# kjeffery/SimplePath

Hardware: AMD Instinct MI355X
Metric: Mrays/sec (+ Msamples/sec) at fixed spp; per-pixel L2 vs CPU ref (higher is better)
Workload: dtype f32; 1 GPU; bunny.sp 1920x1080 @ 256 spp, direct_lighting; width=1920, height=1080, spp=256, integrator=direct_lighting, bvh=sah, tiles=32400, pipeline=megakernel, parallelism=tiles1

## Files before the change

simplepath_amd/csrc/common/sp_libm.h:

```cpp
#pragma once
#include "sp_math.h"
#include "sp_glibc_data.h"

namespace spm {

SP_HD double dfma(double a, double b, double c) { return __builtin_fma(a, b, c); }
SP_HD double gd(const uint64_t* t, int i) { return u2d(t[i]); }

template <uint64_t B>
SP_HD double vk(double dep)
{
#if defined(__HIP_DEVICE_COMPILE__)
    uint32_t lo, hi;
    asm("v_mov_b32 %0, %1 ; %2" : "=v"(lo) : "i"((uint32_t)(B & 0xffffffffull)), "v"(dep));
    asm("v_mov_b32 %0, %1 ; %2" : "=v"(hi) : "i"((uint32_t)(B >> 32)), "v"(dep));
    return u2d(((uint64_t)hi << 32) | (uint64_t)lo);
#else
    (void)dep;
    return u2d(B);
#endif
}

#if defined(__HIP_DEVICE_COMPILE__)
static __shared__ uint64_t lds_exp2f_t[32];
static __shared__ uint64_t lds_logf_t[32];
static __shared__ uint64_t lds_powf_t[32];
__device__ __forceinline__ void libm_lds_init(int tid, int nthreads)
{
    for (int i = tid; i < 32; i += nthreads) {
        lds_exp2f_t[i] = glibc::EXP2F_T[i];
        lds_logf_t[i]  = glibc::LOGF_T[i];
        lds_powf_t[i]  = glibc::POWF_T[i];
    }
}
#define SPM_EXP2F_T lds_exp2f_t
#define SPM_LOGF_T lds_logf_t
#define SPM_POWF_T lds_powf_t
#else
SP_HD void libm_lds_init(int, int) {}
#define SPM_EXP2F_T glibc::EXP2F_T
#define SPM_LOGF_T glibc::LOGF_T
#define SPM_POWF_T glibc::POWF_T
#endif
SP_HD float gf(const uint32_t* t, int i) { return u2f(t[i]); }

SP_HD float x86_default_nan() { return u2f(0xffc00000u); }
SP_HD float x86_quiet(float x) { return u2f(f2u(x) | 0x00400000u); }
SP_HD bool  is_nan_bits(float x) { return (f2u(x) & 0x7fffffffu) > 0x7f800000u; }
SP_HD float x86_add(float a, float b)
{
    if (is_nan_bits(a)) return x86_quiet(a);
    if (is_nan_bits(b)) return x86_quiet(b);
    return a + b;
}

SP_HD float lm_expf(float x)
{
#if defined(SP_XP_FASTLIBM) && defined(__HIP_DEVICE_COMPILE__)
    return __expf(x);
#endif
    using namespace glibc;
    const uint32_t ix     = f2u(x);
    const uint32_t abstop = (ix >> 20) & 0x7ffu;
    const double   xd     = (double)x;
    if (abstop > 0x42au) {
        if (ix == 0xff800000u) return 0.0f;
        if (abstop > 0x7f7u) return x86_add(x, x);
        if (x > gf(EXPF_LIM, 0)) return __builtin_inff();
        if (gf(EXPF_LIM, 1) > x) return 0.0f;
        if (!(gf(EXPF_LIM, 2) <= x)) return u2f(0x00000001u);
    }
    const double invln2n = gd(EXPF_K, 1), shift = gd(EXPF_K, 0);
    double       kd      = dfma(invln2n, xd, shift);
    const uint64_t ki    = d2u(kd);
    kd -= shift;
    const double r = dfma(invln2n, xd, -kd);
    uint64_t     t = SPM_EXP2F_T[ki & 31u] + (ki << 47);
    const double s  = u2d(t);
    const double z  = dfma(r, gd(EXPF_K, 2), vk<EXPF_K[3]>(r));
    const double r2 = r * r;
    double       y  = dfma(r, gd(EXPF_K, 4), gd(ONE_D, 0));
    y               = dfma(z, r2, y);
    y               = y * s;
    return (float)y;
}

SP_HD float lm_logf(float x)
{
#if defined(SP_XP_FASTLIBM) && defined(__HIP_DEVICE_COMPILE__)
    return __logf(x);
#endif
    using namespace glibc;
    uint32_t ix = f2u(x);
    if (ix == 0x3f800000u) return 0.0f;
    if (ix - 0x00800000u > 0x7effffffu) {
        if (ix * 2u == 0u) return -__builtin_inff();
        if (ix == 0x7f800000u) return x;
        if (ix * 2u > 0xfeffffffu) return x86_quiet(x);
        if (ix & 0x80000000u) return x86_default_nan();
        ix = f2u(x * gf(TWO23_F, 0)) - (23u << 23);
    }
    const uint32_t tmp  = ix - 0x3f330000u;
    const uint32_t i    = (tmp >> 19) & 15u;
    const int32_t  k    = (int32_t)tmp >> 23;
    const uint32_t iz   = ix - (tmp & 0xff800000u);
    const double   invc = gd(SPM_LOGF_T, 2 * i), logc = gd(SPM_LOGF_T, 2 * i + 1);
    const double   z    = (double)u2f(iz);
    const double   r    = dfma(z, invc, gd(MINUS_ONE_D, 0));
    const double   y0   = dfma((double)k, gd(LOGF_K, 0), logc);
    const double   r2   = r * r;
    double         y    = dfma(r, gd(LOGF_K, 2), vk<LOGF_K[3]>(r));
    y                   = dfma(r2, gd(LOGF_K, 1), y);
    y                   = dfma(r2, y, r + y0);
    return (float)y;
}

SP_HD int powf_checkint(uint32_t iy)
{
    const int e = (int)((iy >> 23) & 0xffu);
    if (e < 0x7f) return 0;
    if (e > 0x7f + 23) return 2;
    if (iy & ((1u << (0x7f + 23 - e)) - 1u)) return 0;
    if (iy & (1u << (0x7f + 23 - e))) return 1;
    return 2;
}
SP_HD bool powf_zeroinfnan(uint32_t ix) { return 2u * ix - 1u >= 2u * 0x7f800000u - 1u; }
SP_HD bool issignalingf(uint32_t ix) { return ((ix & 0x7fffffffu) > 0x7f800000u) && !(ix & 0x00400000u); }

SP_HD float lm_powf(float x, float y)
{
#if defined(SP_XP_FASTLIBM) && defined(__HIP_DEVICE_COMPILE__)
    return __powf(x, y);
#endif
    using namespace glibc;
    uint32_t       sign_bias = 0;
    uint32_t       ix = f2u(x);
    const uint32_t iy = f2u(y);
    if (ix - 0x00800000u >= 0x7f000000u || powf_zeroinfnan(iy)) {
        if (powf_zeroinfnan(iy)) {
            if (2u * iy == 0u) return issignalingf(ix) ? x86_add(x, y) : 1.0f;
            if (ix == 0x3f800000u) return issignalingf(iy) ? x86_add(x, y) : 1.0f;
            if (2u * ix > 2u * 0x7f800000u || 2u * iy > 2u * 0x7f800000u) return x86_add(x, y);
            if (2u * ix == 2u * 0x3f800000u) return 1.0f;
            if ((2u * ix < 2u * 0x3f800000u) == !(iy & 0x80000000u)) return 0.0f;
            return y * y;
        }
        if (powf_zeroinfnan(ix)) {
            float x2 = x * x;
            if ((ix & 0x80000000u) && powf_checkint(iy) == 1) x2 = -x2;
            return (iy & 0x80000000u) ? 1.0f / x2 : x2;
        }
        if (ix & 0x80000000u) {
            const int yint = powf_checkint(iy);
            if (yint == 0) return x86_default_nan();
            if (yint == 1) sign_bias = 1u << 16;
            ix &= 0x7fffffffu;
        }
        if (ix < 0x00800000u) {
            ix = f2u(x * gf(TWO23_F, 0)) & 0x7fffffffu;
            ix -= 23u << 23;
        }
    }
    const uint32_t tmp  = ix - 0x3f330000u;
    const uint32_t i    = (tmp >> 19) & 15u;
    const uint32_t top  = tmp & 0xff800000u;
    const uint32_t iz   = ix - top;
    const int32_t  k    = (int32_t)top >> 23;
    const double   invc = gd(SPM_POWF_T, 2 * i), logc = gd(SPM_POWF_T, 2 * i + 1);
    const double   z    = (double)u2f(iz);
    const double   r    = dfma(z, invc, gd(MINUS_ONE_D, 0));
    const double   y0   = (double)k + logc;
    const double   r2   = r * r;
    double         yy   = dfma(r, gd(POWF_A, 0), vk<POWF_A[1]>(r));
    const double   p    = dfma(r, gd(POWF_A, 2), vk<POWF_A[3]>(r));
    const double   r4   = r2 * r2;
    double         q    = dfma(r, gd(POWF_A, 4), y0);
    q                   = dfma(r2, p, q);
    yy                  = dfma(yy, r4, q);
    const double ylogx  = (double)y * yy;
    if (((d2u(ylogx) >> 47) & 0xffffu) > 0x80beu) {
        if (ylogx > gd(POWF_LIM, 0)) return sign_bias ? -__builtin_inff() : __builtin_inff();
        if (ylogx > gd(POWF_LIM, 1)) {
            const float one = gf(POWF_FLIM, 1) < 0.0f ? 1.0f : 1.0f;
            (void)one;
        }
        if (!(gd(POWF_LIM, 2) < ylogx)) return sign_bias ? -0.0f : 0.0f;
        if (!(gd(POWF_LIM, 3) <= ylogx)) return u2f(sign_bias ? 0x80000001u : 0x00000001u);
    }
    const double   shift = gd(EXP2F_K, 0);
    double         kd    = ylogx + shift;
    const uint64_t ki    = d2u(kd);
    kd -= shift;
    const double   rr  = ylogx - kd;
    uint64_t       t   = SPM_EXP2F_T[ki & 31u];
    const uint64_t ski = ki + sign_bias;
    t += ski << 47;
    const double s   = u2d(t);
    const double zz  = dfma(rr, gd(EXP2F_K, 1), vk<EXP2F_K[2]>(rr));
    const double rr2 = rr * rr;
    double       res = dfma(rr, gd(EXP2F_K, 3), gd(ONE_D, 0));
    res              = dfma(zz, rr2, res);
    res              = res * s;
    return (float)res;
}

SP_HD double sc(int k) { return gd(glibc::SINCOSF_T, k); }
enum { SC_HPI_INV = 4, SC_HPI = 5, SC_C0 = 6, SC_C1 = 7, SC_S1 = 8, SC_C2 = 9, SC_S2 = 10, SC_C3 = 11, SC_S3 = 12, SC_C4 = 13 };
SP_HD double sincos_sign(int q) { return (q == 1 || q == 2) ? -1.0 : 1.0; }

SP_HD float sincosf_poly(double x, double x2, int tab, int n)
{
    if ((n & 1) == 0) {
        const double s1 = dfma(x2, sc(SC_S3), vk<glibc::SINCOSF_T[SC_S2]>(x2));
        const double x3 = x2 * x;
        const double x7 = x2 * x3;
        const double s  = dfma(x3, sc(SC_S1), x);
        return (float)dfma(s1, x7, s);
    }
    const double x4 = x2 * x2;
    const double c1 = dfma(x2, sc(SC_C1), vk<glibc::SINCOSF_T[SC_C0]>(x2));
    const double c2 = dfma(x2, sc(SC_C4), vk<glibc::SINCOSF_T[SC_C3]>(x2));
    const double x6 = x2 * x4;
    const double c  = dfma(x4, sc(SC_C2), c1);
    const float  r  = (float)dfma(c2, x6, c);
    return tab ? -r : r;
}

SP_HD double sincosf_reduce_large(uint32_t xi, int* np)
{
    const uint32_t* arr   = glibc::INV_PIO4 + ((xi >> 26) & 15u);
    const int       shift = (int)((xi >> 23) & 7u);
    xi                    = (xi & 0xffffffu) | 0x800000u;
    xi <<= shift;
    uint64_t res0 = (uint64_t)(uint32_t)(xi * arr[0]);
    uint64_t res1 = (uint64_t)xi * arr[4];
    uint64_t res2 = (uint64_t)xi * arr[8];
    res0          = (res2 >> 32) | (res0 << 32);
    res0 += res1;
    const uint64_t n = (res0 + (1ull << 61)) >> 62;
    res0 -= n << 62;
    const double x = (double)(int64_t)res0;
    *np            = (int)n;
    return x * u2d(glibc::PI63[0]);
}

template <bool BOUNDED = false>
SP_HD float lm_sinf(float y)
{
#if defined(SP_XP_FASTLIBM) && defined(__HIP_DEVICE_COMPILE__)
    return __sinf(y);
#endif
    const uint32_t iy     = f2u(y);
    const uint32_t abstop = (iy >> 20) & 0x7ffu;
    double         x      = (double)y;
    if (abstop <= 0x3f3u) {
        const double s = x * x;
        if (abstop <= 0x397u) return y;
        return sincosf_poly(x, s, 0, 0);
    }
    if (BOUNDED || abstop <= 0x42eu) {
        const double r  = x * sc(SC_HPI_INV);
        int          n  = (((int32_t)r) + 0x800000) >> 24;
        x               = dfma(-(double)n, sc(SC_HPI), x);
        const double sg = sincos_sign(n & 3);
        const int    tb = (n & 2) ? 1 : 0;
        return sincosf_poly(x * sg, x * x, tb, n);
    }
    if (abstop <= 0x7f7u) {
        const int sign = (int)(iy >> 31);
        int       n;
        x               = sincosf_reduce_large(iy, &n);
        const double sg = sincos_sign((n + sign) & 3);
        const int    tb = ((n + sign) & 2) ? 1 : 0;
        return sincosf_poly(x * sg, x * x, tb, n);
    }
    return ((iy & 0x7fffffffu) > 0x7f800000u) ? x86_quiet(y) : x86_default_nan();
}

template <bool BOUNDED = false>
SP_HD float lm_cosf(float y)
{
#if defined(SP_XP_FASTLIBM) && defined(__HIP_DEVICE_COMPILE__)
    return __cosf(y);
#endif
    const uint32_t iy     = f2u(y);
    const uint32_t abstop = (iy >> 20) & 0x7ffu;
// ... 356 lines not shown
```

simplepath_amd/csrc/common/sp_math.h:

```cpp
#pragma once

#include <stdint.h>
#include <math.h>

#if defined(__HIPCC__)
#include <hip/hip_runtime.h>
#define SP_HD __host__ __device__ __forceinline__
#define SP_DEV __device__ __forceinline__
#else
#define SP_HD static inline
#define SP_DEV static inline
#endif

#if !defined(__HIP_DEVICE_COMPILE__)
#include <immintrin.h>
#endif

namespace spm {

SP_HD uint32_t f2u(float f) { return __builtin_bit_cast(uint32_t, f); }
SP_HD float u2f(uint32_t u) { return __builtin_bit_cast(float, u); }
SP_HD uint64_t d2u(double d) { return __builtin_bit_cast(uint64_t, d); }
SP_HD double u2d(uint64_t u) { return __builtin_bit_cast(double, u); }

SP_HD float std_max(float a, float b) { return (a < b) ? b : a; }
SP_HD float std_min(float a, float b) { return (b < a) ? b : a; }
SP_HD float std_clamp(float v, float lo, float hi) { return (v < lo) ? lo : ((hi < v) ? hi : v); }
SP_HD float sse_min(float a, float b) { return (a < b) ? a : b; }
SP_HD float sse_max(float a, float b) { return (a > b) ? a : b; }
SP_HD float fma_f(float a, float b, float c) { return __builtin_fmaf(a, b, c); }
SP_HD float abs_f(float a) { return __builtin_fabsf(a); }
SP_HD float sqrt_f(float a) { return __builtin_sqrtf(a); }
SP_HD float copysign_f(float a, float b) { return __builtin_copysignf(a, b); }

constexpr float k_pi          = 3.14159265358979323846f;
constexpr float k_inv_pi      = 0.318309886183790671538f;
constexpr float k_ray_epsilon = 0.001f;
constexpr float k_infinite    = 3.40282346638528859812e+38f;

struct RsqrtTable {
    const uint32_t* entries;
    int32_t         bits;
    uint32_t        zero_result;
    uint32_t        denorm_result;
    int32_t  pack_shift = 0;
    uint32_t pack_hi    = 0;
};

SP_HD float rsqrtss_emulated(float x, const RsqrtTable& t)
{
    const uint32_t u = f2u(x);
    const uint32_t e = (u >> 23) & 0xffu;
    if ((u >> 31) != 0u) {
        if ((u & 0x7fffffffu) == 0u) return u2f(0xff800000u);
        if (e == 0xffu && (u & 0x7fffffu) != 0u) return u2f(u | 0x400000u);
        return u2f(0xffc00000u);
    }
    if (e == 0xffu) {
        if ((u & 0x7fffffu) != 0u) return u2f(u | 0x400000u);
        return 0.0f;
    }
    if (e == 0u) {
        if (u == 0u) return u2f(t.zero_result);
        return u2f(t.denorm_result);
    }
    const int32_t  ex   = (int32_t)e - 127;
    const int32_t  p    = ex & 1;
    const int32_t  q    = (ex - p) / 2;
    const uint32_t m    = (u & 0x7fffffu) >> (23 - t.bits);
    const uint32_t i    = ((uint32_t)p << t.bits) | m;
    const uint32_t r    = t.pack_shift ? (t.pack_hi | ((uint32_t)((const uint16_t*)t.entries)[i] << t.pack_shift)) : t.entries[i];
    const int32_t  re   = (int32_t)((r >> 23) & 0xffu) - q;
    return u2f((r & 0x807fffffu) | ((uint32_t)re << 23));
}

SP_HD float rsqrt_newton(float a, float r)
{
    const float t1 = 1.5f * r;
    const float t2 = a * -0.5f;
    const float t3 = t2 * r;
    const float t4 = r * r;
    const float t5 = t3 * t4;
    return t1 + t5;
}

#if !defined(__HIP_DEVICE_COMPILE__)
static inline float rsqrtss_host(float x) { return _mm_cvtss_f32(_mm_rsqrt_ss(_mm_set_ss(x))); }
#else
static inline float rsqrtss_host(float) { return 0.0f; }
#endif

struct f3 {
    float x, y, z;
};

SP_HD f3 mk(float x, float y, float z) { f3 r; r.x = x; r.y = y; r.z = z; return r; }
SP_HD f3 add(f3 a, f3 b) { return mk(a.x + b.x, a.y + b.y, a.z + b.z); }
SP_HD f3 sub(f3 a, f3 b) { return mk(a.x - b.x, a.y - b.y, a.z - b.z); }
SP_HD f3 mul(f3 a, f3 b) { return mk(a.x * b.x, a.y * b.y, a.z * b.z); }
SP_HD f3 scale(f3 a, float s) { return mk(a.x * s, a.y * s, a.z * s); }
SP_HD f3 scale(float s, f3 a) { return mk(s * a.x, s * a.y, s * a.z); }
SP_HD f3 divs(f3 a, float s) { return mk(a.x / s, a.y / s, a.z / s); }
SP_HD f3 neg(f3 a) { return mk(-a.x, -a.y, -a.z); }
SP_HD f3 madd(f3 a, f3 b, f3 c) { return mk(fma_f(a.x, b.x, c.x), fma_f(a.y, b.y, c.y), fma_f(a.z, b.z, c.z)); }
SP_HD f3 madd(float a, f3 b, f3 c) { return mk(fma_f(a, b.x, c.x), fma_f(a, b.y, c.y), fma_f(a, b.z, c.z)); }

SP_HD float dot(f3 a, f3 b)
{
    const float p0 = a.x * b.x;
    const float p1 = a.y * b.y;
    const float p2 = a.z * b.z;
    return (p0 + p1) + (p2 + 0.0f);
}

SP_HD float dop1(float a, float b, float c, float d)
{
    const float cd  = c * d;
    const float err = fma_f(-c, d, cd);
    const float dop = fma_f(a, b, -cd);
    return dop + err;
}

SP_HD f3 cross(f3 a, f3 b)
{
    return mk(dop1(a.y, b.z, a.z, b.y), dop1(a.z, b.x, a.x, b.z), dop1(a.x, b.y, a.y, b.x));
}

SP_HD float length(f3 a) { return sqrt_f(dot(a, a)); }

struct rgb {
    float r, g, b;
};
SP_HD rgb mkc(float r, float g, float b) { rgb c; c.r = r; c.g = g; c.b = b; return c; }
SP_HD rgb cadd(rgb a, rgb b) { return mkc(a.r + b.r, a.g + b.g, a.b + b.b); }
SP_HD rgb csub(rgb a, rgb b) { return mkc(a.r - b.r, a.g - b.g, a.b - b.b); }
SP_HD rgb cmul(rgb a, rgb b) { return mkc(a.r * b.r, a.g * b.g, a.b * b.b); }
SP_HD rgb cscale(rgb a, float s) { return mkc(a.r * s, a.g * s, a.b * s); }
SP_HD rgb cdivs(rgb a, float s) { return mkc(a.r / s, a.g / s, a.b / s); }
SP_HD bool cblack(rgb a) { return a.r == 0.0f && a.g == 0.0f && a.b == 0.0f; }
SP_HD float luminance(rgb c) { return 0.2126f * c.r + 0.7152f * c.g + 0.0722f * c.b; }

struct aff {
    f3 vx, vy, vz, p;
};
struct lin {
    f3 vx, vy, vz;
};

SP_HD f3 xfm_point(const aff& m, f3 p)
{
    return madd(mk(p.x, p.x, p.x), m.vx, madd(mk(p.y, p.y, p.y), m.vy, madd(mk(p.z, p.z, p.z), m.vz, m.p)));
}
SP_HD f3 xfm_vector(const f3& vx, const f3& vy, const f3& vz, f3 a)
{
    return madd(mk(a.x, a.x, a.x), vx, madd(mk(a.y, a.y, a.y), vy, mul(mk(a.z, a.z, a.z), vz)));
}
// ... 5 lines not shown
```

simplepath_amd/csrc/hip/sp_path.hpp:

```cpp
#pragma once
#include "sp_device.hpp"

namespace spd {
inline namespace SPD_LAYOUT_NS {

using namespace spm;

#ifdef SP_WAVE_PROF
static __shared__ unsigned long long wprof_lds[16 * 16];
__device__ __forceinline__ void wprof_end(int k, uint64_t t0)
{
    const uint64_t dt    = __builtin_amdgcn_s_memtime() - t0;
    const uint64_t m     = __ballot(1);
    const int      first = __ffsll((unsigned long long)m) - 1;
    if ((int)(threadIdx.x & 63) == first) {
        const int w = threadIdx.x >> 6;
        wprof_lds[w * 16 + 2 * k] += dt;
        wprof_lds[w * 16 + 2 * k + 1] += dt * (uint64_t)__popcll(m);
    }
}
#define SP_WPROF(k, stmt)                                                                                              \
    do {                                                                                                               \
        const uint64_t t_wp_ = __builtin_amdgcn_s_memtime();                                                           \
        stmt;                                                                                                          \
// ... 1529 lines not shown
    lm_sincosf_bounded(phi, &sp, &cp);
    return mk(r * cp, y, r * sp);
}
__device__ __forceinline__ P2 concentric_disk(P2 u)
{
    constexpr float pi_over_4 = k_pi / 4.0f;
    constexpr float pi_over_2 = k_pi / 2.0f;
    const float     ox = 2.0f * u.x - 1.0f;
    const float     oy = 2.0f * u.y - 1.0f;
    P2              r;
    if (ox == 0.0f && oy == 0.0f) { r.x = 0.0f; r.y = 0.0f; return r; }
    float theta, rad;
    if (abs_f(ox) > abs_f(oy)) { rad = ox; theta = pi_over_4 * (oy / ox); }
    else { rad = oy; theta = pi_over_2 - pi_over_4 * (ox / oy); }
    float st, ct;
    lm_sincosf_bounded(theta, &st, &ct);
    r.x = rad * ct;
    r.y = rad * st;
    return r;
}
__device__ __forceinline__ f3 sample_cosine_hemisphere(P2 u)
{
    const P2    d = concentric_disk(u);
    const float y = sqrt_unit(std_max(0.0f, 1.0f - d.x * d.x - d.y * d.y));
    return mk(d.x, y, d.y);
}
constexpr float k_uniform_sphere_pdf     = 1.0f / (4.0f * k_pi);
constexpr float k_uniform_hemisphere_pdf = 1.0f / (2.0f * k_pi);

struct Onb {
    f3 u, v, w;
};
__device__ __forceinline__ Onb onb_of_unit(f3 v)
{
    const float sign = copysign_f(1.0f, v.z);
    const float a    = -1.0f / (sign + v.z);
    const float b    = v.x * v.y * a;
    const f3    b1   = mk(1.0f + sign * v.x * v.x * a, sign * b, -sign * v.x);
    const f3    b2   = mk(b, sign + v.y * v.y * a, -v.y);
    Onb         o;
    o.u = b2;
    o.v = v;
    o.w = b1;
    return o;
}
__device__ __forceinline__ Onb onb_from_v(f3 n, const Rsq& q) { return onb_of_unit(normalize(n, q)); }
__device__ __forceinline__ f3 to_world(const Onb& o, f3 a) { return add(add(scale(a.x, o.u), scale(a.y, o.v)), scale(a.z, o.w)); }
__device__ __forceinline__ f3 to_onb(const Onb& o, f3 a) { return mk(dot(a, o.u), dot(a, o.v), dot(a, o.w)); }

struct MSample {
    rgb   color;
    f3    dir;
    float pdf;
    int   props;
};
constexpr int PROP_DIFFUSE = 1, PROP_GLOSSY = 2, PROP_SPECULAR = 4, PROP_REFLECTIVE = 8;

__device__ __forceinline__ float cos2_theta(f3 w) { return w.y * w.y; }
__device__ __forceinline__ float sin2_theta(f3 w) { return std_max(0.0f, 1.0f - cos2_theta(w)); }
__device__ __forceinline__ float sin_theta(f3 w) { return sqrt_unit(sin2_theta(w)); }
__device__ __forceinline__ float tan_theta(f3 w) { return sin_theta(w) / w.y; }
__device__ __forceinline__ float tan2_theta(f3 w) { return sin2_theta(w) / cos2_theta(w); }
__device__ __forceinline__ float cos_phi(f3 w)
{
    const float st = sin_theta(w);
    return (st == 0.0f) ? 1.0f : std_clamp(w.x / st, -1.0f, 1.0f);
}
__device__ __forceinline__ float sin_phi(f3 w)
{
    const float st = sin_theta(w);
    return (st == 0.0f) ? 1.0f : std_clamp(w.z / st, -1.0f, 1.0f);
}
__device__ __forceinline__ bool same_hemisphere(f3 a, f3 b) { return a.y * b.y > 0.0f; }

__device__ __forceinline__ float fresnel_dielectric(float cos_i, float eta_i, float eta_t)
{
    cos_i = std_clamp(cos_i, -1.0f, 1.0f);
    if (!(cos_i > 0.0f)) {
        const float s = eta_i; eta_i = eta_t; eta_t = s;
        cos_i = abs_f(cos_i);
    }
    const float sin_i = sqrt_unit(std_max(0.0f, 1.0f - cos_i * cos_i));
    const float sin_t = eta_i / eta_t * sin_i;
    if (sin_t >= 1) return 1.0f;
    const float cos_t = sqrt_unit(std_max(0.0f, 1.0f - sin_t * sin_t));
    const float parl  = ((eta_t * cos_i) - (eta_i * cos_t)) / ((eta_t * cos_i) + (eta_i * cos_t));
    const float perp  = ((eta_i * cos_i) - (eta_t * cos_t)) / ((eta_i * cos_i) + (eta_t * cos_t));
    return (parl * parl + perp * perp) / 2.0f;
}

__device__ __forceinline__ float erfinv(float a)
{
    float       p;
    const float t = lm_logf(fma_f(a, 0.0f - a, 1.0f));
    if (abs_f(t) > 6.125f) {
        p = 3.03697567e-10f;
        p = fma_f(p, t, 2.93243101e-8f);
        p = fma_f(p, t, 1.22150334e-6f);
        p = fma_f(p, t, 2.84108955e-5f);
        p = fma_f(p, t, 3.93552968e-4f);
        p = fma_f(p, t, 3.02698812e-3f);
        p = fma_f(p, t, 4.83185798e-3f);
        p = fma_f(p, t, -2.64646143e-1f);
        p = fma_f(p, t, 8.40016484e-1f);
    } else {
        p = 5.43877832e-9f;
        p = fma_f(p, t, 1.43285448e-7f);
        p = fma_f(p, t, 1.22774793e-6f);
        p = fma_f(p, t, 1.12963626e-7f);
        p = fma_f(p, t, -5.61530760e-5f);
        p = fma_f(p, t, -1.47697632e-4f);
        p = fma_f(p, t, 2.31468678e-3f);
        p = fma_f(p, t, 1.15392581e-2f);
        p = fma_f(p, t, -2.32015476e-1f);
        p = fma_f(p, t, 8.86226892e-1f);
    }
    return a * p;
}

__device__ __forceinline__ P2 beckmann_sample11(float cos_theta_i, float U1, float U2)
{
    P2 s;
    if (cos_theta_i > .9999f) {
        const float r  = sqrt_f(-lm_logf(1.0f - U1));
        float       sp, cp;
        lm_sincosf_bounded(2.0f * k_pi * U2, &sp, &cp);
        s.x = r * cp;
        s.y = r * sp;
        return s;
    }
    const float sin_theta_i = sqrt_unit(std_max(0.0f, 1.0f - cos_theta_i * cos_theta_i));
    const float tan_theta_i = sin_theta_i / cos_theta_i;
    const float cot_theta_i = 1.0f / tan_theta_i;
    float       a           = -1.0f;
    float       c           = lm_erff(cot_theta_i);
    const float sample_x    = std_max(U1, 1e-6f);
    const float theta_i     = lm_acosf(cos_theta_i);
    const float fit         = 1.0f + theta_i * (-0.876f + theta_i * (0.4265f - 0.0594f * theta_i));
    float       b           = c - (1.0f + c) * lm_powf(1.0f - sample_x, fit);
    const float sqrt_pi_inv = 1.0f / sqrt_f(k_pi);
    const float normalization =
        1.0f / (1.0f + c + sqrt_pi_inv * tan_theta_i * lm_expf(-cot_theta_i * cot_theta_i));
#pragma unroll 1
    for (int it = 0; it < 9; ++it) {
        if (!(b >= a && b <= c)) b = 0.5f * (a + c);
        const float inv_erf = erfinv(b);
        const float value =
            normalization * (1.0f + b + sqrt_pi_inv * tan_theta_i * lm_expf(-inv_erf * inv_erf)) - sample_x;
        const float derivative = normalization * (1.0f - inv_erf * tan_theta_i);
        if (abs_f(value) < 1e-5f) break;
        if (value > 0) c = b;
        else a = b;
        b -= value / derivative;
    }
    s.x = erfinv(b);
    s.y = erfinv(2.0f * std_max(U2, 1e-6f) - 1.0f);
    return s;
}

__device__ __forceinline__ f3 beckmann_sample(f3 wi, float ax, float ay, float U1, float U2, const Rsq& q)
{
    const f3 st = normalize(mk(ax * wi.x, wi.y, ay * wi.z), q);
    P2       sl = beckmann_sample11(st.y, U1, U2);
    const float tmp = cos_phi(st) * sl.x - sin_phi(st) * sl.y;
    sl.y            = sin_phi(st) * sl.x + cos_phi(st) * sl.y;
    sl.x            = tmp;
    sl.x            = ax * sl.x;
    sl.y            = ay * sl.y;
    return normalize(mk(-sl.x, 1.0f, -sl.y), q);
}

__device__ __forceinline__ float beck_D(const Material& m, f3 wh)
{
    const float t2 = tan2_theta(wh);
    if (__builtin_isinf(t2)) return 0.0f;
    const float c4 = cos2_theta(wh) * cos2_theta(wh);
    const float cp = cos_phi(wh), sp = sin_phi(wh);
    return lm_expf(-t2 * ((cp * cp) / (m.alpha_x * m.alpha_x) + (sp * sp) / (m.alpha_y * m.alpha_y))) /
           (k_pi * m.alpha_x * m.alpha_y * c4);
}
__device__ __forceinline__ float beck_lambda(const Material& m, f3 w)
{
    const float at = abs_f(tan_theta(w));
    if (__builtin_isinf(at)) return 0.0f;
    const float cp    = cos_phi(w), sp = sin_phi(w);
    const float alpha = sqrt_f((cp * cp) * (m.alpha_x * m.alpha_x) + (sp * sp) * (m.alpha_y * m.alpha_y));
    const float a     = 1.0f / (alpha * at);
    if (a >= 1.6f) return 0.0f;
    return (1.0f - 1.259f * a + 0.396f * (a * a)) / (3.535f * a + 2.181f * (a * a));
}
__device__ __forceinline__ float beck_G1(const Material& m, f3 w) { return 1.0f / (1.0f + beck_lambda(m, w)); }
__device__ __forceinline__ float beck_G(const Material& m, f3 wo, f3 wi) { return 1.0f / (1.0f + beck_lambda(m, wo) + beck_lambda(m, wi)); }
__device__ __forceinline__ float beck_pdf(const Material& m, f3 wo, f3 wh)
{
    if (m.sample_visible_area) return beck_D(m, wh) * beck_G1(m, wo) * abs_f(dot(wo, wh)) / abs_f(wo.y);
    return beck_D(m, wh) * abs_f(wh.y);
}
__device__ __forceinline__ f3 beck_sample_wh(const Material& m, f3 wo, Rng& rng, const Rsq& q)
{
    const bool flip = wo.y < 0.0f;
    const float U2 = next1D(rng);
    const float U1 = next1D(rng);
    f3 wh = beckmann_sample(flip ? neg(wo) : wo, m.alpha_x, m.alpha_y, U1, U2, q);
    if (flip) wh = neg(wh);
    return wh;
}

__device__ __forceinline__ rgb mf_eval(const Material& m, f3 wo, f3 wi, const Rsq& q)
{
    const float ao = abs_f(wo.y), ai = abs_f(wi.y);
    if (ai == 0.0f || ao == 0.0f) return mkc(0, 0, 0);
    f3 wh = add(wi, wo);
    if (wh.x == 0.0f && wh.y == 0.0f && wh.z == 0.0f) return mkc(0, 0, 0);
    wh            = normalize(wh, q);
    const float f = fresnel_dielectric(dot(wi, wh), 1.0f, m.microfacet_ior);
    return cdivs(cscale(cscale(cscale(m.microfacet_r, beck_D(m, wh)), beck_G(m, wo, wi)), f), 4.0f * ai * ao);
}
__device__ __forceinline__ float mf_pdf(const Material& m, f3 wo, f3 wi, const Rsq& q)
{
    if (!same_hemisphere(wo, wi)) return 0.0f;
    const f3 wh = normalize(add(wo, wi), q);
    return beck_pdf(m, wo, wh) / (4.0f * dot(wo, wh));
}
__device__ __forceinline__ MSample mf_sample(const Material& m, f3 wo, Rng& rng, const Rsq& q)
{
    MSample r;
    r.color = mkc(0, 0, 0);
    r.dir   = mk(0, 0, 0);
    r.pdf   = 0.0f;
    r.props = 0;
    if (wo.y == 0.0f) return r;
    const f3    wh = beck_sample_wh(m, wo, rng, q);
    const float dp = dot(wo, wh);
    if (dp < 0.0f) return r;
    const f3 wi = add(neg(wo), scale(2.0f * dot(wo, wh), wh));
    if (!same_hemisphere(wo, wi)) return r;
    r.pdf   = beck_pdf(m, wo, wh) / (4.0f * dp);
    r.color = mf_eval(m, wo, wi, q);
    r.dir   = wi;
    r.props = PROP_GLOSSY | PROP_REFLECTIVE;
    return r;
}
struct BeckPre {
    bool  flip, steep;
    f3    st;
    float cphi, sphi;
    float tan_theta_i, c0, fit, normalization, sqrt_pi_inv;
    float lam_wo;
};
__device__ __forceinline__ BeckPre beck_pre(const Material& m, f3 wo, const Rsq& q)
{
    BeckPre p;
    p.flip               = wo.y < 0.0f;
    const f3 wi          = p.flip ? neg(wo) : wo;
    p.st                 = normalize(mk(m.alpha_x * wi.x, wi.y, m.alpha_y * wi.z), q);
    p.cphi               = cos_phi(p.st);
    p.sphi               = sin_phi(p.st);
    const float cos_t    = p.st.y;
    p.steep              = cos_t > .9999f;
    p.tan_theta_i = p.c0 = p.fit = p.normalization = p.sqrt_pi_inv = 0.0f;
    if (!p.steep) {
        const float sin_theta_i = sqrt_unit(std_max(0.0f, 1.0f - cos_t * cos_t));
        p.tan_theta_i           = sin_theta_i / cos_t;
        const float cot_theta_i = 1.0f / p.tan_theta_i;
        p.c0                    = lm_erff(cot_theta_i);
        const float theta_i     = lm_acosf(cos_t);
        p.fit                   = 1.0f + theta_i * (-0.876f + theta_i * (0.4265f - 0.0594f * theta_i));
        p.sqrt_pi_inv           = 1.0f / sqrt_f(k_pi);
        p.normalization = 1.0f / (1.0f + p.c0 + p.sqrt_pi_inv * p.tan_theta_i * lm_expf(-cot_theta_i * cot_theta_i));
    }
    p.lam_wo = beck_lambda(m, wo);
    return p;
}
__device__ __forceinline__ P2 beckmann_sample11_pre(const BeckPre& p, float U1, float U2)
{
    P2 s;
    if (p.steep) {
        const float r  = sqrt_f(-lm_logf(1.0f - U1));
        float       sp, cp;
        lm_sincosf_bounded(2.0f * k_pi * U2, &sp, &cp);
        s.x = r * cp;
        s.y = r * sp;
        return s;
    }
    float       a        = -1.0f;
    float       c        = p.c0;
    const float sample_x = std_max(U1, 1e-6f);
    float       b        = c - (1.0f + c) * lm_powf(1.0f - sample_x, p.fit);
    float inv_erf   = 0.0f;
    bool  converged = false;
#if defined(SP_WAVE_PROF) && defined(SP_WPROF_NEWTON)
    const uint64_t t_nl = __builtin_amdgcn_s_memtime();
#endif
#pragma unroll 1
    for (int it = 0; it < 9; ++it) {
#if defined(SP_WAVE_PROF) && defined(SP_WPROF_NEWTON)
        const uint64_t t_it = __builtin_amdgcn_s_memtime();
#endif
        if (!(b >= a && b <= c)) b = 0.5f * (a + c);
        inv_erf = erfinv(b);
        const float value =
            p.normalization * (1.0f + b + p.sqrt_pi_inv * p.tan_theta_i * lm_expf(-inv_erf * inv_erf)) - sample_x;
        const float derivative = p.normalization * (1.0f - inv_erf * p.tan_theta_i);
#if defined(SP_WAVE_PROF) && defined(SP_WPROF_NEWTON)
        wprof_end(4, t_it);
#endif
        if (abs_f(value) < 1e-5f) {
            converged = true;
            break;
        }
        if (value > 0) c = b;
        else a = b;
        b -= value / derivative;
    }
#if defined(SP_WAVE_PROF) && defined(SP_WPROF_NEWTON)
    wprof_end(5, t_nl);
#endif
    s.x = converged ? inv_erf : erfinv(b);
    s.y = erfinv(2.0f * std_max(U2, 1e-6f) - 1.0f);
    return s;
}
__device__ __forceinline__ MSample mf_sample_pre_u(const Material& m, const BeckPre& p, f3 wo, uint64_t u2, uint64_t u1,
                                                   const Rsq& q);
template <bool NT = false, bool PAIR = (SP_RNG_PAIR != 0)>
__device__ __forceinline__ MSample mf_sample_pre(const Material& m, const BeckPre& p, f3 wo, Rng& rng, const Rsq& q)
{
    MSample r;
    r.color = mkc(0, 0, 0);
    r.dir   = mk(0, 0, 0);
    r.pdf   = 0.0f;
    r.props = 0;
    if (wo.y == 0.0f) return r;
    uint64_t u2, u1;
    rng_raw2<NT, PAIR>(rng, u2, u1);
    return mf_sample_pre_u(m, p, wo, u2, u1, q);
}
struct MGeom {
    f3    dir;
    float pdf;
    float D, G, F, den;
    bool  valid;
    bool  black;
};
__device__ __forceinline__ MGeom mf_sample_geom(const Material& m, const BeckPre& p, f3 wo, uint64_t u2, uint64_t u1,
                                                const Rsq& q)
{
    MGeom g;
    g.dir   = mk(0, 0, 0);
    g.pdf   = 0.0f;
    g.D = g.G = g.F = 0.0f;
    g.den   = 1.0f;
    g.valid = false;
    g.black = true;
    const float U2 = canonical_from_u64(u2);
    const float U1 = canonical_from_u64(u1);
    P2          sl = beckmann_sample11_pre(p, U1, U2);
    const float tmp = p.cphi * sl.x - p.sphi * sl.y;
    sl.y            = p.sphi * sl.x + p.cphi * sl.y;
    sl.x            = tmp;
    sl.x            = m.alpha_x * sl.x;
    sl.y            = m.alpha_y * sl.y;
    f3 wh = normalize(mk(-sl.x, 1.0f, -sl.y), q);
    if (p.flip) wh = neg(wh);
    const float dp = dot(wo, wh);
    if (dp < 0.0f) return g;
    const f3 wi = add(neg(wo), scale(2.0f * dot(wo, wh), wh));
    if (!same_hemisphere(wo, wi)) return g;
    const float bpdf = m.sample_visible_area ? beck_D(m, wh) * (1.0f / (1.0f + p.lam_wo)) * abs_f(dot(wo, wh)) / abs_f(wo.y)
                                             : beck_D(m, wh) * abs_f(wh.y);
    g.pdf   = bpdf / (4.0f * dp);
    g.dir   = wi;
    g.valid = true;
    const float ao = abs_f(wo.y), ai = abs_f(wi.y);
    if (ai == 0.0f || ao == 0.0f) return g;
    f3 h = add(wi, wo);
    if (h.x == 0.0f && h.y == 0.0f && h.z == 0.0f) return g;
    h       = normalize(h, q);
    g.F     = fresnel_dielectric(dot(wi, h), 1.0f, m.microfacet_ior);
    g.G     = 1.0f / (1.0f + p.lam_wo + beck_lambda(m, wi));
    g.D     = beck_D(m, h);
    g.den   = 4.0f * ai * ao;
    g.black = false;
    return g;
}
__device__ __forceinline__ float mf_geom_channel(const MGeom& g, float R) { return g.black ? 0.0f : (((R * g.D) * g.G) * g.F) / g.den; }
__device__ __forceinline__ MSample mf_sample_pre_u(const Material& m, const BeckPre& p, f3 wo, uint64_t u2, uint64_t u1,
                                                   const Rsq& q)
{
    const MGeom g = mf_sample_geom(m, p, wo, u2, u1, q);
    MSample     r;
    r.color = mkc(0, 0, 0);
    r.dir   = g.dir;
    r.pdf   = g.pdf;
    r.props = 0;
    if (!g.valid) return r;
    r.color = mkc(mf_geom_channel(g, m.microfacet_r.r), mf_geom_channel(g, m.microfacet_r.g), mf_geom_channel(g, m.microfacet_r.b));
    r.props = PROP_GLOSSY | PROP_REFLECTIVE;
    return r;
}
__device__ __forceinline__ void rho_accumulate(rgb& r, const MGeom& g, rgb R, bool grey)
{
    if (!(g.pdf > 0.0f)) return;
    const float ay = abs_f(g.dir.y);
    r.r = r.r + (mf_geom_channel(g, R.r) * ay) / g.pdf;
    if (!grey) {
        r.g = r.g + (mf_geom_channel(g, R.g) * ay) / g.pdf;
        r.b = r.b + (mf_geom_channel(g, R.b) * ay) / g.pdf;
    }
}
#ifndef SP_RHO_ALIGNED
#define SP_RHO_ALIGNED 0
#endif
#ifndef SP_RHO_GREY
#define SP_RHO_GREY 1
#endif
template <bool PAIR = (SP_RNG_PAIR != 0), bool ALIGN = (SP_RHO_ALIGNED != 0), bool TOUCH = (SP_RHO_TOUCH != 0)>
__device__ __forceinline__ rgb mf_rho16(const Material& m, f3 wo, Rng& rng, const Rsq& q)
{
    const BeckPre p = beck_pre(m, wo, q);
    rgb           r = mkc(0, 0, 0);
    const bool grey = SP_RHO_GREY && f2u(m.microfacet_r.r) == f2u(m.microfacet_r.g) && f2u(m.microfacet_r.r) == f2u(m.microfacet_r.b);
    rng_reserve(rng, 32);
#if SP_RHO_TOUCH
    if constexpr (TOUCH) rng_touch(rng, 32, (__attribute__((address_space(3))) void*)rho_rng_sink);
#endif
    if constexpr (ALIGN && MT_BLK % 2 == 0 && RNG_PF == 0 && !SP_XP_SERVED_FREE) {
        if (wo.y == 0.0f) return cdivs(r, (float)16u);
        const int       odd   = rng.idx & 1;
        const uint64_t* cur   = mt_buf(rng, rng.cur);
        const uint64_t* next  = mt_buf(rng, mt_next(rng));
        uint64_t        carry = odd ? cur[mt_off(rng.idx)] : 0ull;
        for (unsigned i = 0; i < 16u; ++i) {
            const int       t = rng.idx + odd + 2 * (int)i;
            const uint64_t* b = (t < MT_N) ? cur + mt_off(t) : next + mt_off(t - MT_N);
            SP_TD(td_lines(rng.td_cat, b, 16));
            const ulonglong2 w  = *reinterpret_cast<const ulonglong2*>(b);
            const uint64_t   w0 = odd ? carry : w.x, w1 = odd ? w.x : w.y;
            carry               = w.y;
            rho_accumulate(r, mf_sample_geom(m, p, wo, mt_temper(w0), mt_temper(w1), q), m.microfacet_r, grey);
        }
        rng_skip_reserved(rng, 32);
        if (grey) r.g = r.b = r.r;
        return cdivs(r, (float)16u);
    }
    for (unsigned i = 0; i < 16u; ++i) {
        if (wo.y == 0.0f) continue;
        uint64_t u2, u1;
        rng_raw2<true, PAIR>(rng, u2, u1);
        rho_accumulate(r, mf_sample_geom(m, p, wo, u2, u1, q), m.microfacet_r, grey);
    }
    if (grey) r.g = r.b = r.r;
    return cdivs(r, (float)16u);
}

#if SP_SERVE_RHO
#ifndef SP_MERGE_QUERIES
#define SP_MERGE_QUERIES 1
#endif
enum : int {
    MQ_O = 0,
    MQ_D3 = 192,
    MQ_T3 = 384,
    MQ_D1 = 448,
    MQ_T1 = 640,
    MQ_BEST = 704,
    MQ_ANY = 832,
    MQ_TB = 896,
    MQ_Q = 960,
    MQ_CNT = 992,
    MQ_WORDS = 996,
    SRV_W = 0, SRV_REQ = 512, SRV_WORDS = 576,
    SRV_WAVE_WORDS = (SP_MERGE_QUERIES && MQ_WORDS > SRV_WORDS) ? MQ_WORDS : SRV_WORDS
};
static_assert(SRV_WAVE_WORDS % 4 == 0 && MQ_BEST % 2 == 0, "u64 LDS atomics need 8-byte alignment");
struct MqLayout {
    enum : int { O = MQ_O, D3 = MQ_D3, T3 = MQ_T3, D1 = MQ_D1, T1 = MQ_T1, BEST = MQ_BEST, AMAX = MQ_BEST, ANY = MQ_ANY,
                 TB = MQ_TB, Q = MQ_Q, CNT = MQ_CNT };
};
#ifndef SP_MQ_SHADOW
#define SP_MQ_SHADOW 1
#endif
static __shared__ __attribute__((aligned(16))) uint32_t srv_lds[4][SRV_WAVE_WORDS];
__device__ __forceinline__ float*   srv_w_at(int wave, int k, int j) { return reinterpret_cast<float*>(&srv_lds[wave][SRV_W + (k * 2 + j) * 64]); }
__device__ __forceinline__ uint8_t* srv_req_of(int wave) { return reinterpret_cast<uint8_t*>(&srv_lds[wave][SRV_REQ]); }
#endif

template <bool PAIR = (SP_RNG_PAIR != 0), bool ALIGN = (SP_RHO_ALIGNED != 0), bool TOUCH = (SP_RHO_TOUCH != 0)>
__device__ __forceinline__ void glossy_weights(const Material& m, f3 wo, Rng& rng, const Rsq& q, float w[2])
{
#if SP_SERVE_RHO
// ... 1007 lines not shown
```

Before: 3737 Mrays/s.

## Make libm and microfacet BSDF paths branchless and add unit-range powf fast path

Rewrites expf, logf, powf and the sqrt table lookup so the main polynomial path always runs, with special-case fixups moved to a rarely taken, expect-annotated tail. It also turns early returns in the Beckmann/Fresnel/microfacet eval, pdf, sample and rho helpers into computed selects, to reduce wavefront divergence. A new lm_powf_unit skips all special-case handling for the Beckmann sampling call sites, where x lies in (0,1). The cost is that every lane now does the full arithmetic even on paths that used to exit early, and the unchecked powf is correct only when the inputs stay in that range.

```diff
diff --git a/simplepath_amd/csrc/common/sp_libm.h b/simplepath_amd/csrc/common/sp_libm.h
--- a/simplepath_amd/csrc/common/sp_libm.h
+++ b/simplepath_amd/csrc/common/sp_libm.h
@@ -63,13 +63,6 @@
     const uint32_t ix     = f2u(x);
     const uint32_t abstop = (ix >> 20) & 0x7ffu;
     const double   xd     = (double)x;
-    if (abstop > 0x42au) {
-        if (ix == 0xff800000u) return 0.0f;
-        if (abstop > 0x7f7u) return x86_add(x, x);
-        if (x > gf(EXPF_LIM, 0)) return __builtin_inff();
-        if (gf(EXPF_LIM, 1) > x) return 0.0f;
-        if (!(gf(EXPF_LIM, 2) <= x)) return u2f(0x00000001u);
-    }
     const double invln2n = gd(EXPF_K, 1), shift = gd(EXPF_K, 0);
     double       kd      = dfma(invln2n, xd, shift);
     const uint64_t ki    = d2u(kd);
@@ -82,24 +75,20 @@
     double       y  = dfma(r, gd(EXPF_K, 4), gd(ONE_D, 0));
     y               = dfma(z, r2, y);
     y               = y * s;
-    return (float)y;
-}
-
-SP_HD float lm_logf(float x)
-{
-#if defined(SP_XP_FASTLIBM) && defined(__HIP_DEVICE_COMPILE__)
-    return __logf(x);
-#endif
-    using namespace glibc;
-    uint32_t ix = f2u(x);
-    if (ix == 0x3f800000u) return 0.0f;
-    if (ix - 0x00800000u > 0x7effffffu) {
-        if (ix * 2u == 0u) return -__builtin_inff();
-        if (ix == 0x7f800000u) return x;
-        if (ix * 2u > 0xfeffffffu) return x86_quiet(x);
-        if (ix & 0x80000000u) return x86_default_nan();
-        ix = f2u(x * gf(TWO23_F, 0)) - (23u << 23);
-    }
+    float res       = (float)y;
+    if (__builtin_expect(abstop > 0x42au, 0)) {
+        if (!(gf(EXPF_LIM, 2) <= x)) res = u2f(0x00000001u);
+        if (gf(EXPF_LIM, 1) > x) res = 0.0f;
+        if (x > gf(EXPF_LIM, 0)) res = __builtin_inff();
+        if (abstop > 0x7f7u) res = is_nan_bits(x) ? x86_quiet(x) : x + x;
+        if (ix == 0xff800000u) res = 0.0f;
+    }
+    return res;
+}
+
+SP_HD float logf_core(uint32_t ix)
+{
+    using namespace glibc;
     const uint32_t tmp  = ix - 0x3f330000u;
     const uint32_t i    = (tmp >> 19) & 15u;
     const int32_t  k    = (int32_t)tmp >> 23;
@@ -114,6 +103,24 @@
     y                   = dfma(r2, y, r + y0);
     return (float)y;
 }
+SP_HD float lm_logf(float x)
+{
+#if defined(SP_XP_FASTLIBM) && defined(__HIP_DEVICE_COMPILE__)
+    return __logf(x);
+#endif
+    using namespace glibc;
+    const uint32_t ix = f2u(x);
+    float          res = logf_core(ix);
+    res                = (ix == 0x3f800000u) ? 0.0f : res;
+    if (__builtin_expect(ix - 0x00800000u > 0x7effffffu, 0)) {
+        res = logf_core(f2u(x * gf(TWO23_F, 0)) - (23u << 23));
+        if (ix & 0x80000000u) res = x86_default_nan();
+        if (ix * 2u > 0xfeffffffu) res = x86_quiet(x);
+        if (ix == 0x7f800000u) res = x;
+        if (ix * 2u == 0u) res = -__builtin_inff();
+    }
+    return res;
+}
 
 SP_HD int powf_checkint(uint32_t iy)
 {
@@ -127,40 +134,42 @@
 SP_HD bool powf_zeroinfnan(uint32_t ix) { return 2u * ix - 1u >= 2u * 0x7f800000u - 1u; }
 SP_HD bool issignalingf(uint32_t ix) { return ((ix & 0x7fffffffu) > 0x7f800000u) && !(ix & 0x00400000u); }
 
-SP_HD float lm_powf(float x, float y)
-{
-#if defined(SP_XP_FASTLIBM) && defined(__HIP_DEVICE_COMPILE__)
-    return __powf(x, y);
-#endif
-    using namespace glibc;
-    uint32_t       sign_bias = 0;
-    uint32_t       ix = f2u(x);
+SP_HD bool powf_special(float x, float y, uint32_t* ixp, uint32_t* sign_bias, float* early)
+{
+    using namespace glibc;
+    uint32_t       ix = *ixp;
     const uint32_t iy = f2u(y);
-    if (ix - 0x00800000u >= 0x7f000000u || powf_zeroinfnan(iy)) {
-        if (powf_zeroinfnan(iy)) {
-            if (2u * iy == 0u) return issignalingf(ix) ? x86_add(x, y) : 1.0f;
-            if (ix == 0x3f800000u) return issignalingf(iy) ? x86_add(x, y) : 1.0f;
-            if (2u * ix > 2u * 0x7f800000u || 2u * iy > 2u * 0x7f800000u) return x86_add(x, y);
-            if (2u * ix == 2u * 0x3f800000u) return 1.0f;
-            if ((2u * ix < 2u * 0x3f800000u) == !(iy & 0x80000000u)) return 0.0f;
-            return y * y;
-        }
-        if (powf_zeroinfnan(ix)) {
-            float x2 = x * x;
-            if ((ix & 0x80000000u) && powf_checkint(iy) == 1) x2 = -x2;
-            return (iy & 0x80000000u) ? 1.0f / x2 : x2;
-        }
-        if (ix & 0x80000000u) {
-            const int yint = powf_checkint(iy);
-            if (yint == 0) return x86_default_nan();
-            if (yint == 1) sign_bias = 1u << 16;
-            ix &= 0x7fffffffu;
-        }
-        if (ix < 0x00800000u) {
-            ix = f2u(x * gf(TWO23_F, 0)) & 0x7fffffffu;
-            ix -= 23u << 23;
-        }
-    }
+    if (powf_zeroinfnan(iy)) {
+        if (2u * iy == 0u) { *early = issignalingf(ix) ? x86_add(x, y) : 1.0f; return true; }
+        if (ix == 0x3f800000u) { *early = issignalingf(iy) ? x86_add(x, y) : 1.0f; return true; }
+        if (2u * ix > 2u * 0x7f800000u || 2u * iy > 2u * 0x7f800000u) { *early = x86_add(x, y); return true; }
+        if (2u * ix == 2u * 0x3f800000u) { *early = 1.0f; return true; }
+        if ((2u * ix < 2u * 0x3f800000u) == !(iy & 0x80000000u)) { *early = 0.0f; return true; }
+        *early = y * y;
+        return true;
+    }
+    if (powf_zeroinfnan(ix)) {
+        float x2 = x * x;
+        if ((ix & 0x80000000u) && powf_checkint(iy) == 1) x2 = -x2;
+        *early = (iy & 0x80000000u) ? 1.0f / x2 : x2;
+        return true;
+    }
+    if (ix & 0x80000000u) {
+        const int yint = powf_checkint(iy);
+        if (yint == 0) { *early = x86_default_nan(); return true; }
+        if (yint == 1) *sign_bias = 1u << 16;
+        ix &= 0x7fffffffu;
+    }
+    if (ix < 0x00800000u) {
+        ix = f2u(x * gf(TWO23_F, 0)) & 0x7fffffffu;
+        ix -= 23u << 23;
+    }
+    *ixp = ix;
+    return false;
+}
+SP_HD double powf_log2(uint32_t ix)
+{
+    using namespace glibc;
     const uint32_t tmp  = ix - 0x3f330000u;
     const uint32_t i    = (tmp >> 19) & 15u;
     const uint32_t top  = tmp & 0xff800000u;
@@ -176,17 +185,11 @@
     const double   r4   = r2 * r2;
     double         q    = dfma(r, gd(POWF_A, 4), y0);
     q                   = dfma(r2, p, q);
-    yy                  = dfma(yy, r4, q);
-    const double ylogx  = (double)y * yy;
-    if (((d2u(ylogx) >> 47) & 0xffffu) > 0x80beu) {
-        if (ylogx > gd(POWF_LIM, 0)) return sign_bias ? -__builtin_inff() : __builtin_inff();
-        if (ylogx > gd(POWF_LIM, 1)) {
-            const float one = gf(POWF_FLIM, 1) < 0.0f ? 1.0f : 1.0f;
-            (void)one;
-        }
-        if (!(gd(POWF_LIM, 2) < ylogx)) return sign_bias ? -0.0f : 0.0f;
-        if (!(gd(POWF_LIM, 3) <= ylogx)) return u2f(sign_bias ? 0x80000001u : 0x00000001u);
-    }
+    return dfma(yy, r4, q);
+}
+SP_HD float powf_exp2(double ylogx, uint32_t sign_bias)
+{
+    using namespace glibc;
     const double   shift = gd(EXP2F_K, 0);
     double         kd    = ylogx + shift;
     const uint64_t ki    = d2u(kd);
@@ -202,6 +205,42 @@
     res              = dfma(zz, rr2, res);
     res              = res * s;
     return (float)res;
+}
+
+SP_HD float lm_powf(float x, float y)
+{
+#if defined(SP_XP_FASTLIBM) && defined(__HIP_DEVICE_COMPILE__)
+    return __powf(x, y);
+#endif
+    using namespace glibc;
+    uint32_t sign_bias = 0;
+    uint32_t ix        = f2u(x);
+    bool     done      = false;
+    float    early     = 0.0f;
+    if (__builtin_expect(ix - 0x00800000u >= 0x7f000000u || powf_zeroinfnan(f2u(y)), 0))
+        done = powf_special(x, y, &ix, &sign_bias, &early);
+    const double ylogx = (double)y * powf_log2(ix);
+    float        res   = powf_exp2(ylogx, sign_bias);
+    if (__builtin_expect(((d2u(ylogx) >> 47) & 0xffffu) > 0x80beu, 0)) {
+        if (!(gd(POWF_LIM, 3) <= ylogx)) res = u2f(sign_bias ? 0x80000001u : 0x00000001u);
+        if (!(gd(POWF_LIM, 2) < ylogx)) res = sign_bias ? -0.0f : 0.0f;
+        if (ylogx > gd(POWF_LIM, 0)) res = sign_bias ? -__builtin_inff() : __builtin_inff();
+    }
+    return done ? early : res;
+}
+
+constexpr uint32_t POWF_UNIT_X_LO = 0x33800000u, POWF_UNIT_X_HI = 0x3f7fffefu;
+constexpr uint32_t POWF_FIT_LO = 0x3ee3e95cu, POWF_FIT_HI = 0x3f7cd99du;
+SP_HD bool lm_powf_unit_claims(float x, float y)
+{
+    return f2u(x) - POWF_UNIT_X_LO <= POWF_UNIT_X_HI - POWF_UNIT_X_LO && f2u(y) - POWF_FIT_LO <= POWF_FIT_HI - POWF_FIT_LO;
+}
+SP_HD float lm_powf_unit(float x, float y)
+{
+#if defined(SP_XP_FASTLIBM) && defined(__HIP_DEVICE_COMPILE__)
+    return __powf(x, y);
+#endif
+    return powf_exp2((double)y * powf_log2(f2u(x)), 0u);
 }
 
 SP_HD double sc(int k) { return gd(glibc::SINCOSF_T, k); }
diff --git a/simplepath_amd/csrc/common/sp_math.h b/simplepath_amd/csrc/common/sp_math.h
--- a/simplepath_amd/csrc/common/sp_math.h
+++ b/simplepath_amd/csrc/common/sp_math.h
@@ -51,19 +51,6 @@
 {
     const uint32_t u = f2u(x);
     const uint32_t e = (u >> 23) & 0xffu;
-    if ((u >> 31) != 0u) {
-        if ((u & 0x7fffffffu) == 0u) return u2f(0xff800000u);
-        if (e == 0xffu && (u & 0x7fffffu) != 0u) return u2f(u | 0x400000u);
-        return u2f(0xffc00000u);
-    }
-    if (e == 0xffu) {
-        if ((u & 0x7fffffu) != 0u) return u2f(u | 0x400000u);
-        return 0.0f;
-    }
-    if (e == 0u) {
-        if (u == 0u) return u2f(t.zero_result);
-        return u2f(t.denorm_result);
-    }
     const int32_t  ex   = (int32_t)e - 127;
     const int32_t  p    = ex & 1;
     const int32_t  q    = (ex - p) / 2;
@@ -71,7 +58,20 @@
     const uint32_t i    = ((uint32_t)p << t.bits) | m;
     const uint32_t r    = t.pack_shift ? (t.pack_hi | ((uint32_t)((const uint16_t*)t.entries)[i] << t.pack_shift)) : t.entries[i];
     const int32_t  re   = (int32_t)((r >> 23) & 0xffu) - q;
-    return u2f((r & 0x807fffffu) | ((uint32_t)re << 23));
+    uint32_t       res  = (r & 0x807fffffu) | ((uint32_t)re << 23);
+    if (__builtin_expect(u - 0x00800000u >= 0x7f000000u, 0)) {
+        const bool nan = e == 0xffu && (u & 0x7fffffu) != 0u;
+        if ((u >> 31) != 0u) {
+            res = 0xffc00000u;
+            if (nan) res = u | 0x400000u;
+            if ((u & 0x7fffffffu) == 0u) res = 0xff800000u;
+        } else if (e == 0xffu) {
+            res = nan ? (u | 0x400000u) : 0u;
+        } else {
+            res = (u == 0u) ? t.zero_result : t.denorm_result;
+        }
+    }
+    return u2f(res);
 }
 
 SP_HD float rsqrt_newton(float a, float r)
diff --git a/simplepath_amd/csrc/hip/sp_path.hpp b/simplepath_amd/csrc/hip/sp_path.hpp
--- a/simplepath_amd/csrc/hip/sp_path.hpp
+++ b/simplepath_amd/csrc/hip/sp_path.hpp
@@ -1635,11 +1635,11 @@
     }
     const float sin_i = sqrt_unit(std_max(0.0f, 1.0f - cos_i * cos_i));
     const float sin_t = eta_i / eta_t * sin_i;
-    if (sin_t >= 1) return 1.0f;
     const float cos_t = sqrt_unit(std_max(0.0f, 1.0f - sin_t * sin_t));
     const float parl  = ((eta_t * cos_i) - (eta_i * cos_t)) / ((eta_t * cos_i) + (eta_i * cos_t));
     const float perp  = ((eta_i * cos_i) - (eta_t * cos_t)) / ((eta_i * cos_i) + (eta_t * cos_t));
-    return (parl * parl + perp * perp) / 2.0f;
+    const float f     = (parl * parl + perp * perp) / 2.0f;
+    return (sin_t >= 1) ? 1.0f : f;
 }
 
 __device__ __forceinline__ float erfinv(float a)
@@ -1690,7 +1690,7 @@
     const float sample_x    = std_max(U1, 1e-6f);
     const float theta_i     = lm_acosf(cos_theta_i);
     const float fit         = 1.0f + theta_i * (-0.876f + theta_i * (0.4265f - 0.0594f * theta_i));
-    float       b           = c - (1.0f + c) * lm_powf(1.0f - sample_x, fit);
+    float       b           = c - (1.0f + c) * lm_powf_unit(1.0f - sample_x, fit);
     const float sqrt_pi_inv = 1.0f / sqrt_f(k_pi);
     const float normalization =
         1.0f / (1.0f + c + sqrt_pi_inv * tan_theta_i * lm_expf(-cot_theta_i * cot_theta_i));
@@ -1726,21 +1726,20 @@
 __device__ __forceinline__ float beck_D(const Material& m, f3 wh)
 {
     const float t2 = tan2_theta(wh);
-    if (__builtin_isinf(t2)) return 0.0f;
     const float c4 = cos2_theta(wh) * cos2_theta(wh);
     const float cp = cos_phi(wh), sp = sin_phi(wh);
-    return lm_expf(-t2 * ((cp * cp) / (m.alpha_x * m.alpha_x) + (sp * sp) / (m.alpha_y * m.alpha_y))) /
-           (k_pi * m.alpha_x * m.alpha_y * c4);
+    const float d  = lm_expf(-t2 * ((cp * cp) / (m.alpha_x * m.alpha_x) + (sp * sp) / (m.alpha_y * m.alpha_y))) /
+                    (k_pi * m.alpha_x * m.alpha_y * c4);
+    return __builtin_isinf(t2) ? 0.0f : d;
 }
 __device__ __forceinline__ float beck_lambda(const Material& m, f3 w)
 {
-    const float at = abs_f(tan_theta(w));
-    if (__builtin_isinf(at)) return 0.0f;
+    const float at    = abs_f(tan_theta(w));
     const float cp    = cos_phi(w), sp = sin_phi(w);
     const float alpha = sqrt_f((cp * cp) * (m.alpha_x * m.alpha_x) + (sp * sp) * (m.alpha_y * m.alpha_y));
     const float a     = 1.0f / (alpha * at);
-    if (a >= 1.6f) return 0.0f;
-    return (1.0f - 1.259f * a + 0.396f * (a * a)) / (3.535f * a + 2.181f * (a * a));
+    const float l     = (1.0f - 1.259f * a + 0.396f * (a * a)) / (3.535f * a + 2.181f * (a * a));
+    return (__builtin_isinf(at) || a >= 1.6f) ? 0.0f : l;
 }
 __device__ __forceinline__ float beck_G1(const Material& m, f3 w) { return 1.0f / (1.0f + beck_lambda(m, w)); }
 __device__ __forceinline__ float beck_G(const Material& m, f3 wo, f3 wi) { return 1.0f / (1.0f + beck_lambda(m, wo) + beck_lambda(m, wi)); }
@@ -1762,18 +1761,18 @@
 __device__ __forceinline__ rgb mf_eval(const Material& m, f3 wo, f3 wi, const Rsq& q)
 {
     const float ao = abs_f(wo.y), ai = abs_f(wi.y);
-    if (ai == 0.0f || ao == 0.0f) return mkc(0, 0, 0);
-    f3 wh = add(wi, wo);
-    if (wh.x == 0.0f && wh.y == 0.0f && wh.z == 0.0f) return mkc(0, 0, 0);
+    f3          wh = add(wi, wo);
+    const bool  black = ai == 0.0f || ao == 0.0f || (wh.x == 0.0f && wh.y == 0.0f && wh.z == 0.0f);
     wh            = normalize(wh, q);
     const float f = fresnel_dielectric(dot(wi, wh), 1.0f, m.microfacet_ior);
-    return cdivs(cscale(cscale(cscale(m.microfacet_r, beck_D(m, wh)), beck_G(m, wo, wi)), f), 4.0f * ai * ao);
+    const rgb   c = cdivs(cscale(cscale(cscale(m.microfacet_r, beck_D(m, wh)), beck_G(m, wo, wi)), f), 4.0f * ai * ao);
+    return mkc(black ? 0.0f : c.r, black ? 0.0f : c.g, black ? 0.0f : c.b);
 }
 __device__ __forceinline__ float mf_pdf(const Material& m, f3 wo, f3 wi, const Rsq& q)
 {
-    if (!same_hemisphere(wo, wi)) return 0.0f;
-    const f3 wh = normalize(add(wo, wi), q);
-    return beck_pdf(m, wo, wh) / (4.0f * dot(wo, wh));
+    const f3    wh = normalize(add(wo, wi), q);
+    const float p  = beck_pdf(m, wo, wh) / (4.0f * dot(wo, wh));
+    return same_hemisphere(wo, wi) ? p : 0.0f;
 }
 __device__ __forceinline__ MSample mf_sample(const Material& m, f3 wo, Rng& rng, const Rsq& q)
 {
@@ -1839,7 +1838,7 @@
     float       a        = -1.0f;
     float       c        = p.c0;
     const float sample_x = std_max(U1, 1e-6f);
-    float       b        = c - (1.0f + c) * lm_powf(1.0f - sample_x, p.fit);
+    float       b        = c - (1.0f + c) * lm_powf_unit(1.0f - sample_x, p.fit);
     float inv_erf   = 0.0f;
     bool  converged = false;
 #if defined(SP_WAVE_PROF) && defined(SP_WPROF_NEWTON)
@@ -1898,13 +1897,7 @@
 __device__ __forceinline__ MGeom mf_sample_geom(const Material& m, const BeckPre& p, f3 wo, uint64_t u2, uint64_t u1,
                                                 const Rsq& q)
 {
-    MGeom g;
-    g.dir   = mk(0, 0, 0);
-    g.pdf   = 0.0f;
-    g.D = g.G = g.F = 0.0f;
-    g.den   = 1.0f;
-    g.valid = false;
-    g.black = true;
+    MGeom       g;
     const float U2 = canonical_from_u64(u2);
     const float U1 = canonical_from_u64(u1);
     P2          sl = beckmann_sample11_pre(p, U1, U2);
@@ -1916,24 +1909,21 @@
     f3 wh = normalize(mk(-sl.x, 1.0f, -sl.y), q);
     if (p.flip) wh = neg(wh);
     const float dp = dot(wo, wh);
-    if (dp < 0.0f) return g;
-    const f3 wi = add(neg(wo), scale(2.0f * dot(wo, wh), wh));
-    if (!same_hemisphere(wo, wi)) return g;
+    const f3    wi = add(neg(wo), scale(2.0f * dot(wo, wh), wh));
+    g.valid        = !(dp < 0.0f) && same_hemisphere(wo, wi);
     const float bpdf = m.sample_visible_area ? beck_D(m, wh) * (1.0f / (1.0f + p.lam_wo)) * abs_f(dot(wo, wh)) / abs_f(wo.y)
                                              : beck_D(m, wh) * abs_f(wh.y);
-    g.pdf   = bpdf / (4.0f * dp);
-    g.dir   = wi;
-    g.valid = true;
+    const float pdf = bpdf / (4.0f * dp);
+    g.pdf   = g.valid ? pdf : 0.0f;
+    g.dir   = mk(g.valid ? wi.x : 0.0f, g.valid ? wi.y : 0.0f, g.valid ? wi.z : 0.0f);
     const float ao = abs_f(wo.y), ai = abs_f(wi.y);
-    if (ai == 0.0f || ao == 0.0f) return g;
-    f3 h = add(wi, wo);
-    if (h.x == 0.0f && h.y == 0.0f && h.z == 0.0f) return g;
+    f3          h  = add(wi, wo);
+    g.black = !g.valid || ai == 0.0f || ao == 0.0f || (h.x == 0.0f && h.y == 0.0f && h.z == 0.0f);
     h       = normalize(h, q);
     g.F     = fresnel_dielectric(dot(wi, h), 1.0f, m.microfacet_ior);
     g.G     = 1.0f / (1.0f + p.lam_wo + beck_lambda(m, wi));
     g.D     = beck_D(m, h);
     g.den   = 4.0f * ai * ao;
-    g.black = false;
     return g;
 }
 __device__ __forceinline__ float mf_geom_channel(const MGeom& g, float R) { return g.black ? 0.0f : (((R * g.D) * g.G) * g.F) / g.den; }
@@ -1953,12 +1943,15 @@
 }
 __device__ __forceinline__ void rho_accumulate(rgb& r, const MGeom& g, rgb R, bool grey)
 {
-    if (!(g.pdf > 0.0f)) return;
-    const float ay = abs_f(g.dir.y);
-    r.r = r.r + (mf_geom_channel(g, R.r) * ay) / g.pdf;
+    const bool  take = g.pdf > 0.0f;
+    const float ay   = abs_f(g.dir.y);
+    const float sr   = r.r + (mf_geom_channel(g, R.r) * ay) / g.pdf;
+    r.r              = take ? sr : r.r;
     if (!grey) {
-        r.g = r.g + (mf_geom_channel(g, R.g) * ay) / g.pdf;
-        r.b = r.b + (mf_geom_channel(g, R.b) * ay) / g.pdf;
+        const float sg = r.g + (mf_geom_channel(g, R.g) * ay) / g.pdf;
+        const float sb = r.b + (mf_geom_channel(g, R.b) * ay) / g.pdf;
+        r.g            = take ? sg : r.g;
+        r.b            = take ? sb : r.b;
     }
 }
 #ifndef SP_RHO_ALIGNED
```

Result: faster. 3978 Mrays/s (median of 6 runs) (+6.5%).
